# sean-lo/OptimalMatrixCompletion.jl

Measured on AMD Instinct MI355X. Metric: B&B node-relaxations/sec, 100x100 k=1, higher is better.
Workload: dtype f64

## Files before the change

include/omc.h:

```cpp
#ifndef OMC_H
#define OMC_H

#include <stdint.h>

#ifdef __cplusplus
extern "C" {
#endif

#define OMC_VERSION 100

#define OMC_OPTIMAL 0
#define OMC_SLOW_PROGRESS 1
#define OMC_TIME_LIMIT 2
#define OMC_INFEASIBLE 3

#define OMC_CUT_LINEAR 0
#define OMC_CUT_LINEAR2 1
#define OMC_CUT_LINEAR3 2
#define OMC_DIR_LEFT 0
#define OMC_DIR_MIDDLE 1
#define OMC_DIR_RIGHT 2
#define OMC_DIR_INNER_LEFT 3
#define OMC_DIR_INNER_RIGHT 4
#define OMC_SMALLEST_1_EIGVEC 1
// ... 192 lines not shown
int omc_last_kernel_stats(omc_instance* h, int64_t* launches , double* ms ,
                          int64_t* units );
#define OMC_HOST_CHECK_WAIT 0
#define OMC_HOST_CHECK_SCAN 1
#define OMC_HOST_LIST 2
#define OMC_HOST_EVENT_DRAIN 3
#define OMC_HOST_HARVEST_FLAGS 4
#define OMC_HOST_HARVEST_ENQUEUE 5
#define OMC_HOST_HARVEST_WAIT 6
#define OMC_HOST_HARVEST_BOOK 7
#define OMC_HOST_SETUP_ENQUEUE 8
#define OMC_HOST_CHECK_TOTAL 9
#define OMC_HOST_HARVEST_TOTAL 10
#define OMC_HOST_ASYNC_HARVESTS 11
#define OMC_HOST_QUIET_INTERVALS 12
#define OMC_HOST_NPHASE 13
int omc_last_host_phases(omc_instance* h, double* ms , int64_t* count );

#ifdef __cplusplus
}
#endif
#endif
```

optimalmatrixcompletion.jl_amd/api.py:

```python
from __future__ import annotations

import atexit
import weakref
import ctypes as C

import numpy as np

from . import _lib, certificate
from ._lib import RelaxParams, OmcError

CUT_TYPES = {"linear": 0, "linear2": 1, "linear3": 2}
DIR_CODES = {"left": 0, "middle": 1, "right": 2, "inner_left": 3, "inner_right": 4}
BREAKPOINTS = {"smallest_1_eigvec": 1, "smallest_2_eigvec": 2}
STATUS_NAMES = {0: "OPTIMAL", 1: "SLOW_PROGRESS", 2: "TIME_LIMIT", 3: "INFEASIBLE"}
KERNEL_CLASSES = ["colprox", "cone", "global", "check", "setup", "small", "accel", "cone_sub", "check_col", "check_build", "harvest",
                  "shor_bigcone", "shor_minors", "shor_cols"]
HOST_PHASES = ["check_wait", "check_scan", "list", "event_drain", "harvest_flags", "harvest_enqueue", "harvest_wait", "harvest_book",
               "setup_enqueue", "check_total", "harvest_total", "async_harvests", "quiet_intervals"]
RESIDENCY_KERNELS = ["k_cone_sub<0>", "k_cone_sub<1>", "k_cone_sub<2>", "k_global", "k_small", "k_colprox_pair", "k_colprox_wide", "k_colprox",
                     "k_cone_ws", "k_cone"]


def default_params(**kw) -> RelaxParams:
    p = RelaxParams()
    _lib.load().omc_relax_params_default(C.byref(p))
    for k_, v in kw.items():
        if not hasattr(p, k_):
            raise TypeError(f"unknown relaxation parameter {k_!r}")
        setattr(p, k_, v)
    return p


def _pack_cuts(nodes, n, k, cut_type):
# ... 335 lines not shown
            return out
        self.stage(nodes, disjunctive_cuts_type, params, U_lower, U_upper, rho_scales, load_from, save_to)
        self.solve()
        return self.fetch(want_Y, want_X, want_Theta)

    def kernel_stats(self):
        nc = len(KERNEL_CLASSES); la = np.zeros(nc, np.int64); ms = np.zeros(nc); un = np.zeros(nc, np.int64)
        _lib.check(self._lib.omc_last_kernel_stats(self._h, _lib.ptr(la), _lib.ptr(ms), _lib.ptr(un)))
        return {KERNEL_CLASSES[i]: dict(launches=int(la[i]), ms=float(ms[i]), units=int(un[i])) for i in range(nc)}

    def host_phases(self):
        if not hasattr(self._lib, "omc_last_host_phases"):
            raise OmcError(-100, "this build of the library has no omc_last_host_phases")
        ms = np.zeros(len(HOST_PHASES)); cnt = np.zeros(len(HOST_PHASES), np.int64)
        _lib.check(self._lib.omc_last_host_phases(self._h, _lib.ptr(ms), _lib.ptr(cnt)))
        return {HOST_PHASES[i]: dict(ms=float(ms[i]), count=int(cnt[i])) for i in range(len(HOST_PHASES))}

    def subspace_stats(self):
        out = np.zeros(8, np.int64)
        _lib.check(self._lib.omc_last_subspace_stats(self._h, _lib.ptr(out)))
        return dict(calls=int(out[0]), power_steps=int(out[1]), fallbacks=int(out[2]), seeds=int(out[3]), fail_positive=int(out[4]),
                    fail_steps=int(out[5]), fail_cholesky=int(out[6]), ritz_passes=int(out[7]))

    def shor_subspace_stats(self):
        out = np.zeros(8, np.int64)
        _lib.check(self._lib.omc_last_shor_subspace_stats(self._h, _lib.ptr(out)))
        return dict(calls=int(out[0]), power_steps=int(out[1]), fallbacks=int(out[2]), seeds=int(out[3]), fail_positive=int(out[4]),
                    fail_steps=int(out[5]), fail_cholesky=int(out[6]), ritz_passes=int(out[7]))

    def kernel_residency(self):
        out = np.zeros(len(RESIDENCY_KERNELS), np.int32)
# ... 293 lines not shown
```

optimalmatrixcompletion.jl_amd/csrc/omc_host.h:

```cpp
#pragma once
#include <hip/hip_runtime.h>
#include <stdint.h>
#include <atomic>
#include <mutex>
#include <string>
#include <thread>
#include <unordered_map>
#include <vector>

#include "omc.h"
#include "omc_device.h"
#include "omc_shor_relax.h"

extern thread_local std::string g_err;
static inline int fail(int code, const std::string& msg) { g_err = msg; return code; }
#define HIPCHK(x)                                                                                         \
  do {                                                                                                    \
    hipError_t e_ = (x);                                                                                  \
    if (e_ != hipSuccess) {                                                                               \
      g_err = std::string(#x) + ": " + hipGetErrorString(e_);                                             \
      return (int)e_ > 0 ? (int)e_ : 999;                                                                 \
    }                                                                                                     \
  } while (0)

// ... 41 lines not shown
  bool cone_512 = false;
  bool dense_proj = false;
  bool host_phases = false;
  bool global_nolds = false;
  bool no_colprox_pair = false;
  bool no_graph = false;
  bool no_subspace = false;
  bool no_ws_split = false;
  bool segv_trace = false;
  bool setup_gram_inline = false;
  bool shor_explicit = false;
  bool shor_no_subspace = false;
  int check_xs = 16;
  int colprox_block_min = 65;
  int cone_multi_min = 1025;
  int graph_max = 16;
  int harvest_async = 1;
  int harvest_async_min_live = 256;
  int shor_select_kb = 1048576;
  int streams = 4;
  int sub_debug = 0;
  int sub_qmax = 24;
  int timing_stride = 1;
  int ws_quiet = 1;
};
struct Knob { const char* name; bool Tuning::*flag; int Tuning::*num; };
inline const Knob OMC_KNOBS[] = {
  {"OMC_ALTMIN_NOLDS", &Tuning::altmin_nolds, nullptr},      {"OMC_COLPROX_NO_XCD", &Tuning::colprox_no_xcd, nullptr},
  {"OMC_CONE_512", &Tuning::cone_512, nullptr},              {"OMC_DENSE_PROJ", &Tuning::dense_proj, nullptr},
  {"OMC_GLOBAL_NOLDS", &Tuning::global_nolds, nullptr},      {"OMC_HOST_PHASES", &Tuning::host_phases, nullptr},
  {"OMC_NO_COLPROX_PAIR", &Tuning::no_colprox_pair, nullptr},
  {"OMC_NO_GRAPH", &Tuning::no_graph, nullptr},              {"OMC_NO_SUBSPACE", &Tuning::no_subspace, nullptr},
  {"OMC_NO_WS_SPLIT", &Tuning::no_ws_split, nullptr},        {"OMC_SEGV_TRACE", &Tuning::segv_trace, nullptr},
  {"OMC_SETUP_GRAM_INLINE", &Tuning::setup_gram_inline, nullptr},
  {"OMC_SHOR_EXPLICIT", &Tuning::shor_explicit, nullptr},    {"OMC_SHOR_NO_SUBSPACE", &Tuning::shor_no_subspace, nullptr},
  {"OMC_COLPROX_BLOCK_MIN", nullptr, &Tuning::colprox_block_min},
  {"OMC_CHECK_XS", nullptr, &Tuning::check_xs},              {"OMC_CONE_MULTI_MIN", nullptr, &Tuning::cone_multi_min},
  {"OMC_GRAPH_MAX", nullptr, &Tuning::graph_max},            {"OMC_SHOR_SELECT_KB", nullptr, &Tuning::shor_select_kb},
  {"OMC_HARVEST_ASYNC", nullptr, &Tuning::harvest_async},    {"OMC_HARVEST_ASYNC_MIN_LIVE", nullptr, &Tuning::harvest_async_min_live},
  {"OMC_WS_QUIET", nullptr, &Tuning::ws_quiet},
  {"OMC_STREAMS", nullptr, &Tuning::streams},
  {"OMC_SUB_DEBUG", nullptr, &Tuning::sub_debug},            {"OMC_SUB_QMAX", nullptr, &Tuning::sub_qmax},
  {"OMC_TIMING_STRIDE", nullptr, &Tuning::timing_stride},
};

struct omc_instance {
  int n = 0, m = 0, k = 0, device = 0, nnz = 0, cmax = 0;
  double gamma = 0, sumA2 = 0;
  std::vector<int> col_ptr, col_idx; std::vector<double> col_val;
  std::vector<double> A; std::vector<uint8_t> mask;
  std::vector<double> Ncnt;
  std::vector<int> row_ptr, row_idx; std::vector<double> row_val;
// ... 46 lines not shown
      scolpart, sminpart, sminpart2, sfroB, svvB, se1, se2, soX, soW, soTh, sbigscr, sXsB, ssubSB, ssubIB;
  long long big_sub_tot[8] = {0};
  struct ShorListKey { int64_t nq = 0, nsoc = 0; uint64_t hlist = 0; std::vector<int64_t> idx, soc; };
  int64_t reserve_shor_nq = 0; int reserve_shor_lists = 0; bool reserve_shor_set = false;
  std::unordered_map<uint64_t, std::vector<int>> sh_byhash; std::vector<ShorListKey> sh_lists;
  int sh_group_cap = 0; size_t sh_int_used = 0, sh_int_cap = 0, sh_byte_used = 0, sh_byte_cap = 0;
  int pool_cap = 0; DevBuf pY, pD1, pD3, pU, palpha, psval, pXs, ptheta, pscal, bwarmL, bwarmS; std::vector<int> warm_load, warm_save;
  struct PoolSig { int kind = 0; int64_t nq = 0, nsoc = 0; uint64_t hlist = 0, hsoc = 0; };
  bool pool_shor = false; int64_t pool_nqmax = 0; DevBuf pShor, pShorHdr, sloadpart;
  std::vector<PoolSig> pool_sig, node_sig; std::mutex sig_mu;
  std::vector<int> save_host;
  bool shor_warm = false;
  int64_t shor_warm_stats[4] = {0, 0, 0, 0};
  int64_t launches[OMC_KERNEL_NCLASS] = {0}; double ms[OMC_KERNEL_NCLASS] = {0}; int64_t units[OMC_KERNEL_NCLASS] = {0};
  size_t nnz_rows() const { return row_idx.size(); }
  std::vector<hipEvent_t> ev_pool[2]; size_t ev_used[2] = {0, 0}; int ev_cur = 0;
  std::vector<int> ev_class[2];
};

bool next_event_pair(omc_instance* h);
int finish_events(omc_instance* h, int pool);
#define TIMED_ON(strm, cls, counted, units_, call)                                                            \
  do {                                                                                                        \
    const int pc_ = h->ev_cur;                                                                                \
    const bool t0_ = next_event_pair(h) && hipEventRecord(h->ev_pool[pc_][h->ev_used[pc_]], strm) == hipSuccess; \
    call;                                                                                                     \
    if (t0_ && hipEventRecord(h->ev_pool[pc_][h->ev_used[pc_] + 1], strm) == hipSuccess) {                    \
      h->ev_used[pc_] += 2; h->ev_class[pc_].push_back(cls);                                                  \
    }                                                                                                         \
    if (counted) { h->launches[cls] += 1; h->units[cls] += (units_); }                                        \
  } while (0)
#define TIMED(cls, units_, call) TIMED_ON(h->stream, cls, true, units_, call)

static constexpr int MAX_SWEEPS = 30;
```

optimalmatrixcompletion.jl_amd/csrc/omc_relax_solve.cpp:

```cpp
#include <algorithm>
#include <chrono>
#include <stdio.h>

#include "omc_host.h"
#include "omc_slots.h"

static_assert(SLOT_HARVEST_NONE == OMC_HARVEST_NONE && SLOT_HARVEST_SYNC == OMC_HARVEST_SYNC && SLOT_HARVEST_ASYNC == OMC_HARVEST_ASYNC, "omc_slots.h restates the plans of omc.h");

bool next_event_pair(omc_instance* h) {
  std::vector<hipEvent_t>& pool = h->ev_pool[h->ev_cur];
  while (pool.size() < h->ev_used[h->ev_cur] + 2) {
    hipEvent_t e;
    if (hipEventCreate(&e) != hipSuccess) return false;
    pool.push_back(e);
  }
  return true;
}

int finish_events(omc_instance* h, int pool) {
  for (size_t i = 0; i + 1 < h->ev_used[pool]; i += 2) {
    float msv = 0.f;
    if (hipEventElapsedTime(&msv, h->ev_pool[pool][i], h->ev_pool[pool][i + 1]) == hipSuccess) h->ms[h->ev_class[pool][i / 2]] += msv;
  }
  h->ev_used[pool] = 0; h->ev_class[pool].clear();
  return 0;
}

namespace {

using Clock = std::chrono::steady_clock;

int sum_sub_stat(int* sub_stat, int S, long long tot[8], hipStream_t s) {
  std::vector<int> ss(8 * (size_t)S);
  HIPCHK(hipMemcpyAsync(ss.data(), sub_stat, sizeof(int) * ss.size(), hipMemcpyDeviceToHost, s));
  HIPCHK(hipStreamSynchronize(s));
  for (int q = 0; q < 8; ++q) tot[q] = 0;
  for (int b = 0; b < S; ++b) for (int q = 0; q < 8; ++q) tot[q] += ss[8 * b + q];
  HIPCHK(hipMemsetAsync(sub_stat, 0, sizeof(int) * ss.size(), s));
  return 0;
}

struct SolveLoop {
  struct CloseGuard { omc_instance* h; ~CloseGuard() { std::lock_guard<std::mutex> lk(h->append_mu); h->append_closed = true; h->ws.Btot = h->Btot_live.load(); h->Btot = h->ws.Btot; if (h->shor_on) h->sh.Btot = h->ws.Btot; } };
  struct GraphGuard { hipGraphExec_t e[2] = {nullptr, nullptr}; ~GraphGuard() { for (int q = 0; q < 2; ++q) if (e[q]) (void)hipGraphExecDestroy(e[q]); } };

  omc_instance* const h;
  CloseGuard close_guard;
  const OmcWS& w; const ShWS& sw; const omc_relax_params& P;
  const Tuning tun;
  const int S, check_every;
  const bool multi, shor;
  const hipStream_t s;
  hipStream_t sm = nullptr, sb = nullptr, sc = nullptr;
  int Btot;
  int* done = nullptr; int* jobs = nullptr;
  SlotBook book;
  std::vector<int> harvested_ids;
  int harvested = 0, it = 0, nlist = 0, flags_cur = 0, list_cur = 0;
  bool timed_out = false;
  int drain_pool = -1;
  bool wait_main = true;
  bool ev_main_set = false;
  bool mw_any = false; int mw_budget[2] = {MAX_SWEEPS, MAX_SWEEPS};
  bool split_solve = false;
  bool quiet = false, quiet_next = false;
  int graph_max = 0, gexec_n = -1; GraphGuard graphs;
  int nrefilled = 0; bool list_pushed = false;
  const Clock::time_point t0; Clock::time_point t_last, t_check;

  explicit SolveLoop(omc_instance* h_)
      : h(h_), close_guard{h_}, w(h_->ws), sw(h_->sh), P(h_->params), tun(h_->tun), S(h_->ws.B), check_every(std::max(1, h_->params.check_every)),
        multi(h_->tun.streams > 1), shor(h_->shor_on), s(h_->stream), Btot(h_->Btot_live.load()),
        book(h_->ws.B, nullptr, nullptr), t0(Clock::now()), t_last(t0), t_check(t0) {}

  void stamp_begin() { t_last = Clock::now(); }
  void stamp(int q) { const auto t = Clock::now(); h->host_ms[q] += std::chrono::duration<double, std::milli>(t - t_last).count(); h->host_cnt[q] += 1; t_last = t; }
  double elapsed() const { return std::chrono::duration<double>(Clock::now() - t0).count(); }

  int image_free(int q) {
    if (h->ev_up_rec[q]) { HIPCHK(hipEventSynchronize(h->ev_up[q])); h->ev_up_rec[q] = false; }
    return 0;
  }
  int push_flags(bool sync) {
    const int q = flags_cur; flags_cur ^= 1;
    { int rc = image_free(q); if (rc) return rc; }
    int* flags = h->pin_flags[q].as<int>();
    book.write_flags(flags);
    HIPCHK(hipMemcpyAsync(w.node_of, flags, sizeof(int) * 3 * (size_t)S, hipMemcpyHostToDevice, s));
    HIPCHK(hipEventRecord(h->ev_up[q], s)); h->ev_up_rec[q] = true;
    if (sync) HIPCHK(hipStreamSynchronize(s));
    return 0;
  }
  int push_list() {
    const int q = list_cur; list_cur ^= 1;
    { int rc = image_free(2 + q); if (rc) return rc; }
    int* alist = h->pin_list[q].as<int>();
    nlist = book.write_list(alist);
    if (nlist) { HIPCHK(hipMemcpyAsync(h->bslotlist.p, alist, sizeof(int) * nlist, hipMemcpyHostToDevice, s)); HIPCHK(hipEventRecord(h->ev_up[2 + q], s)); h->ev_up_rec[2 + q] = true; }
    return 0;
  }

  int gram_launch(int njobs) {
    if (tun.setup_gram_inline || njobs <= 0) return 0;
    for (int q = 0; q < njobs; ++q)
      if (jobs[2 * q] < 0 || jobs[2 * q] >= S || jobs[2 * q + 1] < 0 || jobs[2 * q + 1] >= Btot) return fail(OMC_ERR_ARGUMENT, "omc_relax_solve: k_setup_gram job outside the slots / nodes");
    HIPCHK(hipMemcpyAsync(h->bgramjobs.p, jobs, sizeof(int) * 2 * (size_t)njobs, hipMemcpyHostToDevice, sb));
    TIMED_ON(sb, OMC_KERNEL_SETUP, false, 0, omc_launch_setup_gram(&w, h->bgramjobs.as<int>(), njobs, Btot, sb));
    HIPCHK(hipEventRecord(h->ev_gram, sb)); h->ev_gram_rec = true;
    return 0;
  }
  int gram_jobs_free() {
    if (h->ev_gram_rec) { HIPCHK(hipEventSynchronize(h->ev_gram)); h->ev_gram_rec = false; }
    return 0;
  }
  int gram_join() {
    if (h->ev_gram_rec && sb != s) HIPCHK(hipStreamWaitEvent(s, h->ev_gram, 0));
    return 0;
  }
  int setup_slots(int units) {
    if (shor) omc_shor_launch_setup(&sw, s);
    TIMED(OMC_KERNEL_SETUP, units, omc_launch_setup(&w, s));
    { int rc = gram_join(); if (rc) return rc; }
    mw_budget[0] = mw_budget[1] = MAX_SWEEPS;
    quiet = quiet_next = false;
    return 0;
  }

  int prepare() {
    for (int c = 0; c < OMC_KERNEL_NCLASS; ++c) { h->launches[c] = 0; h->ms[c] = 0; h->units[c] = 0; }
    for (int q = 0; q < 2; ++q) { h->ev_used[q] = 0; h->ev_class[q].clear(); }
    h->ev_cur = 0;
    for (int q = 0; q < OMC_HOST_NPHASE; ++q) { h->host_ms[q] = 0; h->host_cnt[q] = 0; }
    for (int q = 0; q < 2; ++q) { int rc = h->pin_flags[q].ensure(sizeof(int) * 3 * (size_t)S); if (rc) return rc; rc = h->pin_list[q].ensure(sizeof(int) * (size_t)S); if (rc) return rc; }
    { int rc = h->pin_done.ensure(sizeof(int) * ((size_t)S + 1)); if (rc) return rc; rc = h->pin_jobs.ensure(sizeof(int) * 2 * (size_t)S); if (rc) return rc; rc = h->bgramjobs.ensure(sizeof(int) * 2 * (size_t)S); if (rc) return rc; }
    for (int q = 0; q < 4; ++q) { if (!h->ev_up[q]) HIPCHK(hipEventCreateWithFlags(&h->ev_up[q], hipEventDisableTiming)); h->ev_up_rec[q] = false; }
    if (!h->ev_gram) HIPCHK(hipEventCreateWithFlags(&h->ev_gram, hipEventDisableTiming));
    h->ev_gram_rec = false;
    if (multi && !h->ev_main) {
      for (hipStream_t& q : h->gs) HIPCHK(hipStreamCreateWithFlags(&q, hipStreamNonBlocking));
      for (int q = 0; q < 5; ++q) { HIPCHK(hipEventCreateWithFlags(&h->gev[q], hipEventDisableTiming)); HIPCHK(hipEventCreateWithFlags(&h->gevc[q], hipEventDisableTiming)); }
      HIPCHK(hipEventCreateWithFlags(&h->ev_main, hipEventDisableTiming));
    }
    sm = multi ? h->gs[0] : s; sb = multi ? h->gs[1] : s; sc = multi ? h->gs[2] : s;
    h->ws.setup_gram_inline = tun.setup_gram_inline ? 1 : 0;
    h->ws.check_xs = std::min(std::max(0, tun.check_xs), CB_XS);
    done = h->pin_done.as<int>(); jobs = h->pin_jobs.as<int>();
    book = SlotBook(S, jobs, done);
    int rc = gram_launch(book.start(Btot)); if (rc) return rc;
    rc = push_flags(false); if (rc) return rc;
    if (book.active() < S) { HIPCHK(hipMemcpyAsync(w.done, done, sizeof(int) * S, hipMemcpyHostToDevice, s)); HIPCHK(hipStreamSynchronize(s)); }
    rc = setup_slots(S); if (rc) return rc;
    rc = push_list(); if (rc) return rc;
    h->total_sweeps = 0;
    graph_max = Btot <= tun.graph_max ? tun.graph_max : 0;
    mw_any = w.geo.mw || (shor && h->wbig.geo.mw);
    for (int q = 0; q < 5; ++q) h->mw_tot[q] = 0;
    split_solve = multi && !tun.no_ws_split && w.sub_enable && w.geo.ws_lpp && w.ws_first;
    return 0;
// ... 30 lines not shown
    *ended = false;
    {
      std::lock_guard<std::mutex> lk(h->append_mu);
      Btot = h->Btot_live.load();
      if (timed_out) { int rc = close_unslotted(OMC_ST_TIME); if (rc) return rc; }
      if (book.next_node() >= Btot && (!h->hold.load() || elapsed() > P.time_limit)) { h->append_closed = true; *ended = true; return 0; }
    }
    if (book.next_node() >= Btot) { std::this_thread::sleep_for(std::chrono::microseconds(100)); return 0; }
    return refill_idle();
  }

  int enqueue_body(const OmcWS& wg, bool timed, bool with_aa, bool capturing) {
    const int gact = book.running();
    const bool split = split_solve && (capturing || !quiet);
    hipEvent_t* const ev = capturing ? h->gevc : h->gev;
    if (multi) {
      HIPCHK(hipEventRecord(ev[0], sm));
      HIPCHK(hipStreamWaitEvent(sb, ev[0], 0)); HIPCHK(hipStreamWaitEvent(sc, ev[0], 0));
    }
#define MAYBE_TIMED(strm, cls, units_, call) do { if (timed) TIMED_ON(strm, cls, true, units_, call); else { call; } } while (0)
    if (shor) {
      OmcWS wb = h->wbig; wb.nB = wg.nB; wb.slot_list = wg.slot_list;
      if (w.sub_enable) MAYBE_TIMED(sm, OMC_KERNEL_CONESUB, gact, omc_launch_cone_sub(&wg, sm));
      if (wb.sub_enable) MAYBE_TIMED(sb, OMC_KERNEL_SHOR_BIGCONE, 0, omc_launch_cone_sub(&wb, sb));
      wb.mw_budget = mw_budget[1];
      if (wb.geo.ws_lpp || wb.geo.mw) MAYBE_TIMED(sb, OMC_KERNEL_SHOR_BIGCONE, gact, omc_launch_cone_ws(&wb, sb));
      else MAYBE_TIMED(sb, OMC_KERNEL_SHOR_BIGCONE, gact, omc_launch_cone(&wb, CONE_BIG, sb));
      if (w.geo.ws_lpp || w.geo.mw) MAYBE_TIMED(sm, OMC_KERNEL_CONE, gact, omc_launch_cone_ws(&wg, sm));
      else MAYBE_TIMED(sm, OMC_KERNEL_CONE, gact, omc_launch_cone(&wg, CONE_CLIP01, sm));
      MAYBE_TIMED(sc, OMC_KERNEL_SMALL, gact, omc_launch_small(&wg, SMALL_PROJ, sc));
      MAYBE_TIMED(sc, OMC_KERNEL_SHOR_MINORS, gact, { omc_shor_launch_minor_pre(&sw, sc); omc_shor_launch_vkeys(&sw, sc); });
      if (multi) {
        HIPCHK(hipEventRecord(ev[1], sb)); HIPCHK(hipEventRecord(ev[2], sc));
        HIPCHK(hipStreamWaitEvent(sm, ev[1], 0)); HIPCHK(hipStreamWaitEvent(sm, ev[2], 0));
      }
      MAYBE_TIMED(sm, OMC_KERNEL_GLOBAL, gact, omc_launch_global(&wg, sm));
      MAYBE_TIMED(sm, OMC_KERNEL_SHOR_COLS, gact, omc_shor_launch_cols(&sw, sm));
      MAYBE_TIMED(sm, OMC_KERNEL_SHOR_MINORS, gact, { omc_shor_launch_minor_post(&sw, sm); omc_shor_launch_reduce(&sw, sm); });
      return 0;
    }
    if (split) {
      MAYBE_TIMED(sc, OMC_KERNEL_SMALL, gact, omc_launch_small(&wg, SMALL_PROJ, sc));
      OmcWS wA = wg; wA.ws_phase = 1;
      MAYBE_TIMED(sc, OMC_KERNEL_CONE, gact, omc_launch_cone_ws(&wA, sc));
      HIPCHK(hipEventRecord(ev[4], sc));
    }
    if (w.sub_enable) MAYBE_TIMED(sm, OMC_KERNEL_CONESUB, gact, omc_launch_cone_sub(&wg, sm));
    MAYBE_TIMED(sb, OMC_KERNEL_COLPROX, (int64_t)gact * w.m, omc_launch_colprox(&wg, 0, sb));
    if (split) {
      HIPCHK(hipStreamWaitEvent(sm, ev[4], 0));
      OmcWS wB = wg; wB.ws_phase = 2;
      MAYBE_TIMED(sm, OMC_KERNEL_CONE, 0, omc_launch_cone_ws(&wB, sm));
    }
    else if (w.geo.ws_lpp || w.geo.mw) MAYBE_TIMED(sm, OMC_KERNEL_CONE, gact, omc_launch_cone_ws(&wg, sm));
    else MAYBE_TIMED(sm, OMC_KERNEL_CONE, gact, omc_launch_cone(&wg, CONE_CLIP01, sm));
    if (!split) MAYBE_TIMED(sc, OMC_KERNEL_SMALL, gact, omc_launch_small(&wg, SMALL_PROJ, sc));
    if (multi) {
      HIPCHK(hipEventRecord(ev[1], sb)); HIPCHK(hipEventRecord(ev[2], sc));
      HIPCHK(hipStreamWaitEvent(sm, ev[1], 0)); HIPCHK(hipStreamWaitEvent(sm, ev[2], 0));
    }
    MAYBE_TIMED(sm, OMC_KERNEL_GLOBAL, gact, omc_launch_global(&wg, sm));
    if (with_aa) MAYBE_TIMED(sm, OMC_KERNEL_ACCEL, gact, omc_launch_aa(&wg, sm));
#undef MAYBE_TIMED
    return 0;
  }

  int capture_body(const OmcWS& wg) {
    hipGraphExec_t* const gexec = graphs.e;
    for (int q = 0; q < 2; ++q) { if (gexec[q]) { (void)hipGraphExecDestroy(gexec[q]); gexec[q] = nullptr; } }
    for (int q = 0; q < (w.accel ? 2 : 1); ++q) {
      hipGraph_t gr = nullptr;
      HIPCHK(hipStreamBeginCapture(sm, hipStreamCaptureModeThreadLocal));
      int rc = enqueue_body(wg, false, q == 1, true);
      hipError_t ce = hipStreamEndCapture(sm, &gr);
      if (rc) { if (gr) (void)hipGraphDestroy(gr); return rc; }
      HIPCHK(ce);
      hipError_t ie = hipGraphInstantiate(&gexec[q], gr, nullptr, nullptr, 0);
      (void)hipGraphDestroy(gr);
      HIPCHK(ie);
    }
    gexec_n = nlist;
    return 0;
  }

  int enqueue_iteration(bool* is_check) {
    ++it;
    *is_check = (it % check_every == 0);
    if (multi && wait_main && !ev_main_set) HIPCHK(hipEventRecord(h->ev_main, s));
    ev_main_set = false;
    const bool sampled = tun.timing_stride > 0 && (it % tun.timing_stride) == 0;
    const bool use_graph = multi && nlist <= graph_max && !tun.no_graph && !(sampled && tun.timing_stride > 1) && !mw_any;
    if (book.running() > 0) {
      OmcWS wg = w; wg.slot_list = h->bslotlist.as<int>(); wg.nB = nlist; wg.mw_budget = mw_budget[0];
      if (multi && wait_main) HIPCHK(hipStreamWaitEvent(sm, h->ev_main, 0));
      if (use_graph) {
        if (gexec_n != nlist) { int rc = capture_body(wg); if (rc) return rc; }
        HIPCHK(hipGraphLaunch(graphs.e[(!*is_check && w.accel) ? 1 : 0], sm));
        h->launches[OMC_KERNEL_GLOBAL] += 1; h->units[OMC_KERNEL_GLOBAL] += book.running();
      } else {
        if (quiet && split_solve && (it - 1) % check_every == 0) h->host_cnt[OMC_HOST_QUIET_INTERVALS] += 1;
        int rc = enqueue_body(wg, sampled, !*is_check && w.accel, false); if (rc) return rc;
      }
      if (multi && *is_check) { HIPCHK(hipEventRecord(h->gev[3], sm)); HIPCHK(hipStreamWaitEvent(s, h->gev[3], 0)); }
    }
    wait_main = false;
    if (drain_pool >= 0) {
      stamp_begin(); finish_events(h, drain_pool); drain_pool = -1; stamp(OMC_HOST_EVENT_DRAIN);
    }
    return 0;
  }

  void enqueue_check() {
    const int nactive = book.active();
    wait_main = true;
    timed_out = elapsed() > P.time_limit;
    TIMED(OMC_KERNEL_CHECK_COL, nactive, {
      if (shor) omc_shor_launch_check(&sw, s);
      else { omc_launch_check_zero(&w, s); omc_launch_colprox(&w, 1, s); }
    });
    TIMED(OMC_KERNEL_CHECK_BUILD, nactive, omc_launch_check_build(&w, s));
    TIMED(OMC_KERNEL_CHECK, nactive, {
      if (w.cert_enable) {
        omc_launch_cert_sub(&w, s);
        omc_launch_check_final(&w, timed_out ? OMC_ST_TIME : 0, 0, s);
        OmcWS wc = w; wc.ws_mode = 1; omc_launch_cone_ws(&wc, s);
        omc_launch_check_final(&w, timed_out ? OMC_ST_TIME : 0, 1, s);
      } else {
        if (w.geo.ws_lpp || w.geo.mw) { OmcWS wc = w; wc.ws_mode = 1; omc_launch_cone_ws(&wc, s); }
        else omc_launch_cone(&w, CONE_EVALS, s);
// ... 23 lines not shown
    return 0;
  }

  int read_check() {
    stamp_begin();
    const bool track_quiet = split_solve && tun.ws_quiet && w.ws_need;
    done[S] = 1;
    HIPCHK(hipMemcpyAsync(done, w.done, sizeof(int) * ((size_t)S + (track_quiet ? 1 : 0)), hipMemcpyDeviceToHost, s));
    if (track_quiet) HIPCHK(hipMemsetAsync(w.ws_need, 0, sizeof(int), s));
    HIPCHK(hipStreamSynchronize(s));
    stamp(OMC_HOST_CHECK_WAIT);
    quiet_next = track_quiet && done[S] == 0;
    t_check = t_last;
    nrefilled = 0; list_pushed = false;
    { int rc = mw_collect(); if (rc) return rc; }
    if (drain_pool >= 0) { finish_events(h, drain_pool); drain_pool = -1; }
    drain_pool = h->ev_cur; h->ev_cur ^= 1;
    Btot = h->Btot_live.load();
    if (!P.first_wins) return 0;
    std::vector<int> stv(S);
    HIPCHK(hipMemcpyAsync(stv.data(), w.status, sizeof(int) * S, hipMemcpyDeviceToHost, s));
    HIPCHK(hipStreamSynchronize(s));
    bool won = false;
    for (int b = 0; b < S; ++b) if (book.node(b) >= 0 && done[b] && stv[b] == OMC_ST_OPTIMAL) won = true;
    if (!won) return 0;
    book.finish_all();
    HIPCHK(hipMemcpyAsync(w.done, done, sizeof(int) * S, hipMemcpyHostToDevice, s));
    HIPCHK(hipStreamSynchronize(s));
    return close_unslotted(OMC_ST_SLOW);
  }

  void enqueue_harvest(int nslots) {
    TIMED(OMC_KERNEL_HARVEST, nslots, {
      if (w.save_to) omc_launch_state_save(&w, s);
      if (shor) omc_shor_launch_state_save(&sw, s);
      omc_launch_small(&w, SMALL_RECOVER, s);
      if (w.sep_done) omc_launch_sep_sub(&w, s);
      omc_launch_cone(&w, CONE_SEP, s);
      omc_launch_harvest(&w, s);
      if (w.cert_flag) omc_launch_cert_harvest(&w, s);
      if (shor) omc_shor_launch_harvest(&sw, s);
    });
  }
  void book_harvested() {
    if (w.save_to) {
      std::lock_guard<std::mutex> lk(h->sig_mu);
      for (int id : harvested_ids) {
// ... 12 lines not shown
    nrefilled = book.book_async(Btot, timed_out, harvested_ids);
    book_harvested();
    stamp(OMC_HOST_HARVEST_BOOK);
    rc = gram_launch(nrefilled); if (rc) return rc;
    rc = push_flags(false); if (rc) return rc;
    if (nrefilled) { rc = setup_slots(nrefilled); if (rc) return rc; }
    stamp(OMC_HOST_SETUP_ENQUEUE);
    return 0;
  }

  int harvest_async() {
    const int npend = book.mark_async();
    int rc = push_list(); if (rc) return rc;
    list_pushed = true;
    stamp(OMC_HOST_LIST);
    if (multi) { HIPCHK(hipEventRecord(h->ev_main, s)); ev_main_set = true; }
    rc = push_flags(false); if (rc) return rc;
    stamp(OMC_HOST_HARVEST_FLAGS);
    enqueue_harvest(npend);
    stamp(OMC_HOST_HARVEST_ENQUEUE);
    h->host_cnt[OMC_HOST_ASYNC_HARVESTS] += 1;
    return 0;
  }

  int harvest_sync(int nfin) {
    int rc = gram_jobs_free(); if (rc) return rc;
    rc = gram_launch(book.mark_sync(Btot, timed_out)); if (rc) return rc;
    rc = push_flags(false); if (rc) return rc;
    stamp(OMC_HOST_HARVEST_FLAGS);
    enqueue_harvest(nfin);
    stamp(OMC_HOST_HARVEST_ENQUEUE);
// ... 16 lines not shown
    if (timed_out) { int rc = close_unslotted(OMC_ST_TIME); if (rc) return rc; }
    const int q = harvested_now ? OMC_HOST_HARVEST_TOTAL : OMC_HOST_CHECK_TOTAL;
    h->host_ms[q] += std::chrono::duration<double, std::milli>(Clock::now() - t_check).count(); h->host_cnt[q] += 1;
    return 0;
  }

  int collect_statistics() {
    { int rc = mw_collect(); if (rc) return rc; }
    std::vector<int> sweeps(S);
    HIPCHK(hipMemcpyAsync(sweeps.data(), w.sweeps, sizeof(int) * S, hipMemcpyDeviceToHost, s));
    HIPCHK(hipStreamSynchronize(s));
    for (int v : sweeps) h->total_sweeps += v;
    { int rc = sum_sub_stat(w.sub_stat, S, h->sub_tot, s); if (rc) return rc; }
    if (shor && h->wbig.sub_enable) { int rc = sum_sub_stat(h->wbig.sub_stat, S, h->big_sub_tot, s); if (rc) return rc; }
    HIPCHK(hipGetLastError());
    if (drain_pool >= 0) finish_events(h, drain_pool);
    finish_events(h, h->ev_cur);
    h->last_solve_seconds = elapsed();
    h->last_iters_total = it;
    if (tun.host_phases) {
      static const char* const nm[OMC_HOST_NPHASE] = {"check_wait", "check_scan", "list", "event_drain", "harvest_flags", "harvest_enqueue", "harvest_wait", "harvest_book", "setup_enqueue", "check_total", "harvest_total", "async_harvests", "quiet_intervals"};
      fprintf(stderr, "omc host phases (solve %.1f ms, %d iterations):", 1e3 * h->last_solve_seconds, it);
      for (int q = 0; q < OMC_HOST_NPHASE; ++q) fprintf(stderr, " %s %.3f ms / %lld", nm[q], h->host_ms[q], (long long)h->host_cnt[q]);
      fprintf(stderr, "\n");
    }
    return 0;
  }
};

}

extern "C" {

int omc_cone_multi_budget(int interval_max) { return interval_max > 0 ? std::min(MAX_SWEEPS, interval_max + 2) : MAX_SWEEPS; }

int omc_harvest_plan(int nlive, int nfin, int pending, int check_index, int async_min_live) {
// ... 34 lines not shown
```

Measured before the change: 2265.

## Reuse timing events as cross-stream dependency events via an event tape

Adds an EventTape that tracks the most recent timing event recorded on each stream. Cross-stream joins (fork, side joins, check dependency) wait on that existing event instead of recording a separate sync event, whenever no work has been enqueued on the stream since. This aims to cut the number of hipEventRecord and hipStreamWaitEvent calls per iteration in timed, non-graph bodies. It adds bookkeeping that must call touch() after every enqueue; a missed touch would produce a wrong dependency.

```diff
diff --git a/include/omc.h b/include/omc.h
--- a/include/omc.h
+++ b/include/omc.h
@@ -230,7 +230,9 @@
 #define OMC_HOST_HARVEST_TOTAL 10
 #define OMC_HOST_ASYNC_HARVESTS 11
 #define OMC_HOST_QUIET_INTERVALS 12
-#define OMC_HOST_NPHASE 13
+#define OMC_HOST_BODY_RECORDS 13
+#define OMC_HOST_BODY_WAITS 14
+#define OMC_HOST_NPHASE 15
 int omc_last_host_phases(omc_instance* h, double* ms , int64_t* count );
 
 #ifdef __cplusplus
diff --git a/optimalmatrixcompletion.jl_amd/api.py b/optimalmatrixcompletion.jl_amd/api.py
--- a/optimalmatrixcompletion.jl_amd/api.py
+++ b/optimalmatrixcompletion.jl_amd/api.py
@@ -16,7 +16,8 @@
 KERNEL_CLASSES = ["colprox", "cone", "global", "check", "setup", "small", "accel", "cone_sub", "check_col", "check_build", "harvest",
                   "shor_bigcone", "shor_minors", "shor_cols"]
 HOST_PHASES = ["check_wait", "check_scan", "list", "event_drain", "harvest_flags", "harvest_enqueue", "harvest_wait", "harvest_book",
-               "setup_enqueue", "check_total", "harvest_total", "async_harvests", "quiet_intervals"]
+               "setup_enqueue", "check_total", "harvest_total", "async_harvests", "quiet_intervals", "body_records", "body_waits"]
+HOST_BODY_COUNTS = ("body_records", "body_waits")
 RESIDENCY_KERNELS = ["k_cone_sub<0>", "k_cone_sub<1>", "k_cone_sub<2>", "k_global", "k_small", "k_colprox_pair", "k_colprox_wide", "k_colprox",
                      "k_cone_ws", "k_cone"]
 
@@ -382,7 +383,14 @@
             raise OmcError(-100, "this build of the library has no omc_last_host_phases")
         ms = np.zeros(len(HOST_PHASES)); cnt = np.zeros(len(HOST_PHASES), np.int64)
         _lib.check(self._lib.omc_last_host_phases(self._h, _lib.ptr(ms), _lib.ptr(cnt)))
-        return {HOST_PHASES[i]: dict(ms=float(ms[i]), count=int(cnt[i])) for i in range(len(HOST_PHASES))}
+        return {HOST_PHASES[i]: dict(ms=float(ms[i]), count=int(cnt[i])) for i in range(len(HOST_PHASES)) if HOST_PHASES[i] not in HOST_BODY_COUNTS}
+
+    def event_counts(self):
+        if not hasattr(self._lib, "omc_last_host_phases"):
+            raise OmcError(-100, "this build of the library has no omc_last_host_phases")
+        ms = np.zeros(len(HOST_PHASES)); cnt = np.zeros(len(HOST_PHASES), np.int64)
+        _lib.check(self._lib.omc_last_host_phases(self._h, _lib.ptr(ms), _lib.ptr(cnt)))
+        return {name[len("body_"):]: int(cnt[HOST_PHASES.index(name)]) for name in HOST_BODY_COUNTS}
 
     def subspace_stats(self):
         out = np.zeros(8, np.int64)
diff --git a/optimalmatrixcompletion.jl_amd/csrc/omc_events.h b/optimalmatrixcompletion.jl_amd/csrc/omc_events.h
--- /dev/null
+++ b/optimalmatrixcompletion.jl_amd/csrc/omc_events.h
@@ -0,0 +1,56 @@
+#pragma once
+#include <vector>
+
+template <class Backend>
+class EventTape {
+ public:
+  struct Ev { int pool = -1, index = -1; bool valid() const { return index >= 0; } };
+  struct Launch { int start, stop, cls; };
+
+  EventTape(Backend* be_, int nstreams, bool merge_) : be(be_), merge(merge_), adj(nstreams, -1) {}
+
+  void touch(int stream) { adj[stream] = -1; }
+
+  Ev mark(int stream) {
+    if (merge && adj[stream] >= 0) return Ev{cur, adj[stream]};
+    return fresh(stream);
+  }
+  Ev begin(int stream) { return mark(stream); }
+  Ev end(int stream) { return fresh(stream); }
+
+  bool wait(int stream, Ev e) {
+    const bool ok = be->wait(stream, e.pool, e.index);
+    if (ok) { touch(stream); ++nwaits; }
+    return ok;
+  }
+
+  void launch(Ev start, Ev stop, int cls) { timed[cur].push_back(Launch{start.index, stop.index, cls}); }
+
+  int current() const { return cur; }
+  void swap() { cur ^= 1; for (int& a : adj) a = -1; }
+  const std::vector<Launch>& launches(int pool) const { return timed[pool]; }
+  void drain(int pool) { timed[pool].clear(); used[pool] = 0; if (pool == cur) for (int& a : adj) a = -1; }
+  void reset() { drain(0); drain(1); cur = 0; nrecords = nwaits = 0; }
+
+  long long records() const { return nrecords; }
+  long long waits() const { return nwaits; }
+  void count_record() { ++nrecords; }
+  void count_wait() { ++nwaits; }
+
+ private:
+  Ev fresh(int stream) {
+    const int i = used[cur];
+    if (!be->record(cur, i, stream)) return Ev{};
+    used[cur] = i + 1; ++nrecords;
+    adj[stream] = i;
+    return Ev{cur, i};
+  }
+
+  Backend* be;
+  bool merge;
+  int cur = 0;
+  int used[2] = {0, 0};
+  std::vector<int> adj;
+  std::vector<Launch> timed[2];
+  long long nrecords = 0, nwaits = 0;
+};
diff --git a/optimalmatrixcompletion.jl_amd/csrc/omc_host.h b/optimalmatrixcompletion.jl_amd/csrc/omc_host.h
--- a/optimalmatrixcompletion.jl_amd/csrc/omc_host.h
+++ b/optimalmatrixcompletion.jl_amd/csrc/omc_host.h
@@ -79,6 +79,7 @@
   int check_xs = 16;
   int colprox_block_min = 65;
   int cone_multi_min = 1025;
+  int event_merge = 1;
   int graph_max = 16;
   int harvest_async = 1;
   int harvest_async_min_live = 256;
@@ -101,6 +102,7 @@
   {"OMC_SHOR_EXPLICIT", &Tuning::shor_explicit, nullptr},    {"OMC_SHOR_NO_SUBSPACE", &Tuning::shor_no_subspace, nullptr},
   {"OMC_COLPROX_BLOCK_MIN", nullptr, &Tuning::colprox_block_min},
   {"OMC_CHECK_XS", nullptr, &Tuning::check_xs},              {"OMC_CONE_MULTI_MIN", nullptr, &Tuning::cone_multi_min},
+  {"OMC_EVENT_MERGE", nullptr, &Tuning::event_merge},
   {"OMC_GRAPH_MAX", nullptr, &Tuning::graph_max},            {"OMC_SHOR_SELECT_KB", nullptr, &Tuning::shor_select_kb},
   {"OMC_HARVEST_ASYNC", nullptr, &Tuning::harvest_async},    {"OMC_HARVEST_ASYNC_MIN_LIVE", nullptr, &Tuning::harvest_async_min_live},
   {"OMC_WS_QUIET", nullptr, &Tuning::ws_quiet},
@@ -177,22 +179,7 @@
   int64_t shor_warm_stats[4] = {0, 0, 0, 0};
   int64_t launches[OMC_KERNEL_NCLASS] = {0}; double ms[OMC_KERNEL_NCLASS] = {0}; int64_t units[OMC_KERNEL_NCLASS] = {0};
   size_t nnz_rows() const { return row_idx.size(); }
-  std::vector<hipEvent_t> ev_pool[2]; size_t ev_used[2] = {0, 0}; int ev_cur = 0;
-  std::vector<int> ev_class[2];
+  std::vector<hipEvent_t> ev_pool[2];
 };
 
-bool next_event_pair(omc_instance* h);
-int finish_events(omc_instance* h, int pool);
-#define TIMED_ON(strm, cls, counted, units_, call)                                                            \
-  do {                                                                                                        \
-    const int pc_ = h->ev_cur;                                                                                \
-    const bool t0_ = next_event_pair(h) && hipEventRecord(h->ev_pool[pc_][h->ev_used[pc_]], strm) == hipSuccess; \
-    call;                                                                                                     \
-    if (t0_ && hipEventRecord(h->ev_pool[pc_][h->ev_used[pc_] + 1], strm) == hipSuccess) {                    \
-      h->ev_used[pc_] += 2; h->ev_class[pc_].push_back(cls);                                                  \
-    }                                                                                                         \
-    if (counted) { h->launches[cls] += 1; h->units[cls] += (units_); }                                        \
-  } while (0)
-#define TIMED(cls, units_, call) TIMED_ON(h->stream, cls, true, units_, call)
-
 static constexpr int MAX_SWEEPS = 30;
diff --git a/optimalmatrixcompletion.jl_amd/csrc/omc_relax_solve.cpp b/optimalmatrixcompletion.jl_amd/csrc/omc_relax_solve.cpp
--- a/optimalmatrixcompletion.jl_amd/csrc/omc_relax_solve.cpp
+++ b/optimalmatrixcompletion.jl_amd/csrc/omc_relax_solve.cpp
@@ -2,29 +2,11 @@
 #include <chrono>
 #include <stdio.h>
 
+#include "omc_events.h"
 #include "omc_host.h"
 #include "omc_slots.h"
 
 static_assert(SLOT_HARVEST_NONE == OMC_HARVEST_NONE && SLOT_HARVEST_SYNC == OMC_HARVEST_SYNC && SLOT_HARVEST_ASYNC == OMC_HARVEST_ASYNC, "omc_slots.h restates the plans of omc.h");
-
-bool next_event_pair(omc_instance* h) {
-  std::vector<hipEvent_t>& pool = h->ev_pool[h->ev_cur];
-  while (pool.size() < h->ev_used[h->ev_cur] + 2) {
-    hipEvent_t e;
-    if (hipEventCreate(&e) != hipSuccess) return false;
-    pool.push_back(e);
-  }
-  return true;
-}
-
-int finish_events(omc_instance* h, int pool) {
-  for (size_t i = 0; i + 1 < h->ev_used[pool]; i += 2) {
-    float msv = 0.f;
-    if (hipEventElapsedTime(&msv, h->ev_pool[pool][i], h->ev_pool[pool][i + 1]) == hipSuccess) h->ms[h->ev_class[pool][i / 2]] += msv;
-  }
-  h->ev_used[pool] = 0; h->ev_class[pool].clear();
-  return 0;
-}
 
 namespace {
 
@@ -40,6 +22,32 @@
   return 0;
 }
 
+enum { T_S = 0, T_M = 1, T_B = 2, T_C = 3, T_NSTREAM = 4 };
+struct HipEvents {
+  omc_instance* h; hipStream_t st[T_NSTREAM] = {}; hipError_t last = hipSuccess;
+  bool record(int pool, int i, int stream) {
+    std::vector<hipEvent_t>& p = h->ev_pool[pool];
+    while (p.size() <= (size_t)i) {
+      hipEvent_t e;
+      if ((last = hipEventCreate(&e)) != hipSuccess) return false;
+      p.push_back(e);
+    }
+    return (last = hipEventRecord(p[i], st[stream])) == hipSuccess;
+  }
+  bool wait(int stream, int pool, int i) { return (last = hipStreamWaitEvent(st[stream], h->ev_pool[pool][i], 0)) == hipSuccess; }
+};
+using Tape = EventTape<HipEvents>;
+
+#define TIMED_ON(id, cls, counted, units_, call)                                                          \
+  do {                                                                                                    \
+    const Tape::Ev t0_ = tape.begin(id);                                                                  \
+    call;                                                                                                 \
+    tape.touch(id);                                                                                       \
+    if (t0_.valid()) { const Tape::Ev t1_ = tape.end(id); if (t1_.valid()) tape.launch(t0_, t1_, cls); }  \
+    if (counted) { h->launches[cls] += 1; h->units[cls] += (units_); }                                    \
+  } while (0)
+#define TIMED(cls, units_, call) TIMED_ON(T_S, cls, true, units_, call)
+
 struct SolveLoop {
   struct CloseGuard { omc_instance* h; ~CloseGuard() { std::lock_guard<std::mutex> lk(h->append_mu); h->append_closed = true; h->ws.Btot = h->Btot_live.load(); h->Btot = h->ws.Btot; if (h->shor_on) h->sh.Btot = h->ws.Btot; } };
   struct GraphGuard { hipGraphExec_t e[2] = {nullptr, nullptr}; ~GraphGuard() { for (int q = 0; q < 2; ++q) if (e[q]) (void)hipGraphExecDestroy(e[q]); } };
@@ -52,6 +60,8 @@
   const bool multi, shor;
   const hipStream_t s;
   hipStream_t sm = nullptr, sb = nullptr, sc = nullptr;
+  int im = T_S, ib = T_S, ic = T_S;
+  HipEvents hip_events; Tape tape;
   int Btot;
   int* done = nullptr; int* jobs = nullptr;
   SlotBook book;
@@ -70,12 +80,46 @@
 
   explicit SolveLoop(omc_instance* h_)
       : h(h_), close_guard{h_}, w(h_->ws), sw(h_->sh), P(h_->params), tun(h_->tun), S(h_->ws.B), check_every(std::max(1, h_->params.check_every)),
-        multi(h_->tun.streams > 1), shor(h_->shor_on), s(h_->stream), Btot(h_->Btot_live.load()),
-        book(h_->ws.B, nullptr, nullptr), t0(Clock::now()), t_last(t0), t_check(t0) {}
+        multi(h_->tun.streams > 1), shor(h_->shor_on), s(h_->stream),
+        hip_events{h_}, tape(&hip_events, T_NSTREAM, h_->tun.event_merge != 0), Btot(h_->Btot_live.load()), book(h_->ws.B, nullptr, nullptr), t0(Clock::now()), t_last(t0), t_check(t0) {}
 
   void stamp_begin() { t_last = Clock::now(); }
   void stamp(int q) { const auto t = Clock::now(); h->host_ms[q] += std::chrono::duration<double, std::milli>(t - t_last).count(); h->host_cnt[q] += 1; t_last = t; }
   double elapsed() const { return std::chrono::duration<double>(Clock::now() - t0).count(); }
+
+  void finish_events(int pool) {
+    for (const Tape::Launch& l : tape.launches(pool)) {
+      float msv = 0.f;
+      if (hipEventElapsedTime(&msv, h->ev_pool[pool][l.start], h->ev_pool[pool][l.stop]) == hipSuccess) h->ms[l.cls] += msv;
+    }
+    tape.drain(pool);
+  }
+
+  int depend(int from, int to, int to2, bool on_tape, hipEvent_t fb, bool counted = true) {
+    if (on_tape) {
+      const Tape::Ev e = tape.mark(from);
+      if (e.valid()) {
+        if (!tape.wait(to, e) || (to2 >= 0 && !tape.wait(to2, e))) HIPCHK(hip_events.last);
+        return 0;
+      }
+    }
+    HIPCHK(hipEventRecord(fb, hip_events.st[from])); tape.touch(from); if (counted) tape.count_record();
+    HIPCHK(hipStreamWaitEvent(hip_events.st[to], fb, 0)); tape.touch(to); if (counted) tape.count_wait();
+    if (to2 >= 0) { HIPCHK(hipStreamWaitEvent(hip_events.st[to2], fb, 0)); tape.touch(to2); if (counted) tape.count_wait(); }
+    return 0;
+  }
+  int join_sides(bool on_tape, hipEvent_t fb_b, hipEvent_t fb_c, bool counted) {
+    Tape::Ev eb, ec;
+    if (on_tape) eb = tape.mark(ib);
+    if (!eb.valid()) { HIPCHK(hipEventRecord(fb_b, sb)); tape.touch(ib); if (counted) tape.count_record(); }
+    if (on_tape) ec = tape.mark(ic);
+    if (!ec.valid()) { HIPCHK(hipEventRecord(fb_c, sc)); tape.touch(ic); if (counted) tape.count_record(); }
+    if (eb.valid()) { if (!tape.wait(im, eb)) HIPCHK(hip_events.last); }
+    else { HIPCHK(hipStreamWaitEvent(sm, fb_b, 0)); tape.touch(im); if (counted) tape.count_wait(); }
+    if (ec.valid()) { if (!tape.wait(im, ec)) HIPCHK(hip_events.last); }
+    else { HIPCHK(hipStreamWaitEvent(sm, fb_c, 0)); tape.touch(im); if (counted) tape.count_wait(); }
+    return 0;
+  }
 
   int image_free(int q) {
     if (h->ev_up_rec[q]) { HIPCHK(hipEventSynchronize(h->ev_up[q])); h->ev_up_rec[q] = false; }
@@ -87,6 +131,7 @@
     int* flags = h->pin_flags[q].as<int>();
     book.write_flags(flags);
     HIPCHK(hipMemcpyAsync(w.node_of, flags, sizeof(int) * 3 * (size_t)S, hipMemcpyHostToDevice, s));
+    tape.touch(T_S);
     HIPCHK(hipEventRecord(h->ev_up[q], s)); h->ev_up_rec[q] = true;
     if (sync) HIPCHK(hipStreamSynchronize(s));
     return 0;
@@ -96,6 +141,7 @@
     { int rc = image_free(2 + q); if (rc) return rc; }
     int* alist = h->pin_list[q].as<int>();
     nlist = book.write_list(alist);
+    tape.touch(T_S);
     if (nlist) { HIPCHK(hipMemcpyAsync(h->bslotlist.p, alist, sizeof(int) * nlist, hipMemcpyHostToDevice, s)); HIPCHK(hipEventRecord(h->ev_up[2 + q], s)); h->ev_up_rec[2 + q] = true; }
     return 0;
   }
@@ -105,8 +151,10 @@
     for (int q = 0; q < njobs; ++q)
       if (jobs[2 * q] < 0 || jobs[2 * q] >= S || jobs[2 * q + 1] < 0 || jobs[2 * q + 1] >= Btot) return fail(OMC_ERR_ARGUMENT, "omc_relax_solve: k_setup_gram job outside the slots / nodes");
     HIPCHK(hipMemcpyAsync(h->bgramjobs.p, jobs, sizeof(int) * 2 * (size_t)njobs, hipMemcpyHostToDevice, sb));
-    TIMED_ON(sb, OMC_KERNEL_SETUP, false, 0, omc_launch_setup_gram(&w, h->bgramjobs.as<int>(), njobs, Btot, sb));
+    tape.touch(ib);
+    TIMED_ON(ib, OMC_KERNEL_SETUP, false, 0, omc_launch_setup_gram(&w, h->bgramjobs.as<int>(), njobs, Btot, sb));
     HIPCHK(hipEventRecord(h->ev_gram, sb)); h->ev_gram_rec = true;
+    tape.touch(ib);
     return 0;
   }
   int gram_jobs_free() {
@@ -114,10 +162,11 @@
     return 0;
   }
   int gram_join() {
-    if (h->ev_gram_rec && sb != s) HIPCHK(hipStreamWaitEvent(s, h->ev_gram, 0));
+    if (h->ev_gram_rec && sb != s) { HIPCHK(hipStreamWaitEvent(s, h->ev_gram, 0)); tape.touch(T_S); }
     return 0;
   }
   int setup_slots(int units) {
+    tape.touch(T_S);
     if (shor) omc_shor_launch_setup(&sw, s);
     TIMED(OMC_KERNEL_SETUP, units, omc_launch_setup(&w, s));
     { int rc = gram_join(); if (rc) return rc; }
@@ -128,8 +177,7 @@
 
   int prepare() {
     for (int c = 0; c < OMC_KERNEL_NCLASS; ++c) { h->launches[c] = 0; h->ms[c] = 0; h->units[c] = 0; }
-    for (int q = 0; q < 2; ++q) { h->ev_used[q] = 0; h->ev_class[q].clear(); }
-    h->ev_cur = 0;
+    tape.reset();
     for (int q = 0; q < OMC_HOST_NPHASE; ++q) { h->host_ms[q] = 0; h->host_cnt[q] = 0; }
     for (int q = 0; q < 2; ++q) { int rc = h->pin_flags[q].ensure(sizeof(int) * 3 * (size_t)S); if (rc) return rc; rc = h->pin_list[q].ensure(sizeof(int) * (size_t)S); if (rc) return rc; }
     { int rc = h->pin_done.ensure(sizeof(int) * ((size_t)S + 1)); if (rc) return rc; rc = h->pin_jobs.ensure(sizeof(int) * 2 * (size_t)S); if (rc) return rc; rc = h->bgramjobs.ensure(sizeof(int) * 2 * (size_t)S); if (rc) return rc; }
@@ -142,6 +190,8 @@
       HIPCHK(hipEventCreateWithFlags(&h->ev_main, hipEventDisableTiming));
     }
     sm = multi ? h->gs[0] : s; sb = multi ? h->gs[1] : s; sc = multi ? h->gs[2] : s;
+    if (multi) { im = T_M; ib = T_B; ic = T_C; }
+    hip_events.st[T_S] = s; hip_events.st[T_M] = sm; hip_events.st[T_B] = sb; hip_events.st[T_C] = sc;
     h->ws.setup_gram_inline = tun.setup_gram_inline ? 1 : 0;
     h->ws.check_xs = std::min(std::max(0, tun.check_xs), CB_XS);
     done = h->pin_done.as<int>(); jobs = h->pin_jobs.as<int>();
@@ -202,53 +252,49 @@
     const int gact = book.running();
     const bool split = split_solve && (capturing || !quiet);
     hipEvent_t* const ev = capturing ? h->gevc : h->gev;
-    if (multi) {
-      HIPCHK(hipEventRecord(ev[0], sm));
-      HIPCHK(hipStreamWaitEvent(sb, ev[0], 0)); HIPCHK(hipStreamWaitEvent(sc, ev[0], 0));
-    }
-#define MAYBE_TIMED(strm, cls, units_, call) do { if (timed) TIMED_ON(strm, cls, true, units_, call); else { call; } } while (0)
+    const bool tp = timed && !capturing && tun.event_merge;
+    const bool cnt = !capturing;
+    if (multi) { int rc = depend(im, ib, ic, tp, ev[0], cnt); if (rc) return rc; }
+#define MAYBE_TIMED(id, cls, units_, call) do { if (timed) TIMED_ON(id, cls, true, units_, call); else { call; tape.touch(id); } } while (0)
     if (shor) {
       OmcWS wb = h->wbig; wb.nB = wg.nB; wb.slot_list = wg.slot_list;
-      if (w.sub_enable) MAYBE_TIMED(sm, OMC_KERNEL_CONESUB, gact, omc_launch_cone_sub(&wg, sm));
-      if (wb.sub_enable) MAYBE_TIMED(sb, OMC_KERNEL_SHOR_BIGCONE, 0, omc_launch_cone_sub(&wb, sb));
+      if (w.sub_enable) MAYBE_TIMED(im, OMC_KERNEL_CONESUB, gact, omc_launch_cone_sub(&wg, sm));
+      if (wb.sub_enable) MAYBE_TIMED(ib, OMC_KERNEL_SHOR_BIGCONE, 0, omc_launch_cone_sub(&wb, sb));
       wb.mw_budget = mw_budget[1];
-      if (wb.geo.ws_lpp || wb.geo.mw) MAYBE_TIMED(sb, OMC_KERNEL_SHOR_BIGCONE, gact, omc_launch_cone_ws(&wb, sb));
-      else MAYBE_TIMED(sb, OMC_KERNEL_SHOR_BIGCONE, gact, omc_launch_cone(&wb, CONE_BIG, sb));
-      if (w.geo.ws_lpp || w.geo.mw) MAYBE_TIMED(sm, OMC_KERNEL_CONE, gact, omc_launch_cone_ws(&wg, sm));
-      else MAYBE_TIMED(sm, OMC_KERNEL_CONE, gact, omc_launch_cone(&wg, CONE_CLIP01, sm));
-      MAYBE_TIMED(sc, OMC_KERNEL_SMALL, gact, omc_launch_small(&wg, SMALL_PROJ, sc));
-      MAYBE_TIMED(sc, OMC_KERNEL_SHOR_MINORS, gact, { omc_shor_launch_minor_pre(&sw, sc); omc_shor_launch_vkeys(&sw, sc); });
-      if (multi) {
-        HIPCHK(hipEventRecord(ev[1], sb)); HIPCHK(hipEventRecord(ev[2], sc));
-        HIPCHK(hipStreamWaitEvent(sm, ev[1], 0)); HIPCHK(hipStreamWaitEvent(sm, ev[2], 0));
-      }
-      MAYBE_TIMED(sm, OMC_KERNEL_GLOBAL, gact, omc_launch_global(&wg, sm));
-      MAYBE_TIMED(sm, OMC_KERNEL_SHOR_COLS, gact, omc_shor_launch_cols(&sw, sm));
-      MAYBE_TIMED(sm, OMC_KERNEL_SHOR_MINORS, gact, { omc_shor_launch_minor_post(&sw, sm); omc_shor_launch_reduce(&sw, sm); });
+      if (wb.geo.ws_lpp || wb.geo.mw) MAYBE_TIMED(ib, OMC_KERNEL_SHOR_BIGCONE, gact, omc_launch_cone_ws(&wb, sb));
+      else MAYBE_TIMED(ib, OMC_KERNEL_SHOR_BIGCONE, gact, omc_launch_cone(&wb, CONE_BIG, sb));
+      if (w.geo.ws_lpp || w.geo.mw) MAYBE_TIMED(im, OMC_KERNEL_CONE, gact, omc_launch_cone_ws(&wg, sm));
+      else MAYBE_TIMED(im, OMC_KERNEL_CONE, gact, omc_launch_cone(&wg, CONE_CLIP01, sm));
+      MAYBE_TIMED(ic, OMC_KERNEL_SMALL, gact, omc_launch_small(&wg, SMALL_PROJ, sc));
+      MAYBE_TIMED(ic, OMC_KERNEL_SHOR_MINORS, gact, { omc_shor_launch_minor_pre(&sw, sc); omc_shor_launch_vkeys(&sw, sc); });
+      if (multi) { int rc = join_sides(tp, ev[1], ev[2], cnt); if (rc) return rc; }
+      MAYBE_TIMED(im, OMC_KERNEL_GLOBAL, gact, omc_launch_global(&wg, sm));
+      MAYBE_TIMED(im, OMC_KERNEL_SHOR_COLS, gact, omc_shor_launch_cols(&sw, sm));
+      MAYBE_TIMED(im, OMC_KERNEL_SHOR_MINORS, gact, { omc_shor_launch_minor_post(&sw, sm); omc_shor_launch_reduce(&sw, sm); });
       return 0;
     }
+    Tape::Ev e4;
     if (split) {
-      MAYBE_TIMED(sc, OMC_KERNEL_SMALL, gact, omc_launch_small(&wg, SMALL_PROJ, sc));
+      MAYBE_TIMED(ic, OMC_KERNEL_SMALL, gact, omc_launch_small(&wg, SMALL_PROJ, sc));
       OmcWS wA = wg; wA.ws_phase = 1;
-      MAYBE_TIMED(sc, OMC_KERNEL_CONE, gact, omc_launch_cone_ws(&wA, sc));
-      HIPCHK(hipEventRecord(ev[4], sc));
-    }
-    if (w.sub_enable) MAYBE_TIMED(sm, OMC_KERNEL_CONESUB, gact, omc_launch_cone_sub(&wg, sm));
-    MAYBE_TIMED(sb, OMC_KERNEL_COLPROX, (int64_t)gact * w.m, omc_launch_colprox(&wg, 0, sb));
+      MAYBE_TIMED(ic, OMC_KERNEL_CONE, gact, omc_launch_cone_ws(&wA, sc));
+      if (tp) e4 = tape.mark(ic);
+      if (!e4.valid()) { HIPCHK(hipEventRecord(ev[4], sc)); tape.touch(ic); if (cnt) tape.count_record(); }
+    }
+    if (w.sub_enable) MAYBE_TIMED(im, OMC_KERNEL_CONESUB, gact, omc_launch_cone_sub(&wg, sm));
+    MAYBE_TIMED(ib, OMC_KERNEL_COLPROX, (int64_t)gact * w.m, omc_launch_colprox(&wg, 0, sb));
     if (split) {
-      HIPCHK(hipStreamWaitEvent(sm, ev[4], 0));
+      if (e4.valid()) { if (!tape.wait(im, e4)) HIPCHK(hip_events.last); }
+      else { HIPCHK(hipStreamWaitEvent(sm, ev[4], 0)); tape.touch(im); if (cnt) tape.count_wait(); }
       OmcWS wB = wg; wB.ws_phase = 2;
-      MAYBE_TIMED(sm, OMC_KERNEL_CONE, 0, omc_launch_cone_ws(&wB, sm));
-    }
-    else if (w.geo.ws_lpp || w.geo.mw) MAYBE_TIMED(sm, OMC_KERNEL_CONE, gact, omc_launch_cone_ws(&wg, sm));
-    else MAYBE_TIMED(sm, OMC_KERNEL_CONE, gact, omc_launch_cone(&wg, CONE_CLIP01, sm));
-    if (!split) MAYBE_TIMED(sc, OMC_KERNEL_SMALL, gact, omc_launch_small(&wg, SMALL_PROJ, sc));
-    if (multi) {
-      HIPCHK(hipEventRecord(ev[1], sb)); HIPCHK(hipEventRecord(ev[2], sc));
-      HIPCHK(hipStreamWaitEvent(sm, ev[1], 0)); HIPCHK(hipStreamWaitEvent(sm, ev[2], 0));
-    }
-    MAYBE_TIMED(sm, OMC_KERNEL_GLOBAL, gact, omc_launch_global(&wg, sm));
-    if (with_aa) MAYBE_TIMED(sm, OMC_KERNEL_ACCEL, gact, omc_launch_aa(&wg, sm));
+      MAYBE_TIMED(im, OMC_KERNEL_CONE, 0, omc_launch_cone_ws(&wB, sm));
+    }
+    else if (w.geo.ws_lpp || w.geo.mw) MAYBE_TIMED(im, OMC_KERNEL_CONE, gact, omc_launch_cone_ws(&wg, sm));
+    else MAYBE_TIMED(im, OMC_KERNEL_CONE, gact, omc_launch_cone(&wg, CONE_CLIP01, sm));
+    if (!split) MAYBE_TIMED(ic, OMC_KERNEL_SMALL, gact, omc_launch_small(&wg, SMALL_PROJ, sc));
+    if (multi) { int rc = join_sides(tp, ev[1], ev[2], cnt); if (rc) return rc; }
+    MAYBE_TIMED(im, OMC_KERNEL_GLOBAL, gact, omc_launch_global(&wg, sm));
+    if (with_aa) MAYBE_TIMED(im, OMC_KERNEL_ACCEL, gact, omc_launch_aa(&wg, sm));
 #undef MAYBE_TIMED
     return 0;
   }
@@ -274,26 +320,30 @@
   int enqueue_iteration(bool* is_check) {
     ++it;
     *is_check = (it % check_every == 0);
-    if (multi && wait_main && !ev_main_set) HIPCHK(hipEventRecord(h->ev_main, s));
+    if (multi && wait_main && !ev_main_set) { HIPCHK(hipEventRecord(h->ev_main, s)); tape.touch(T_S); }
     ev_main_set = false;
+    const long long nrec0 = tape.records(), nwait0 = tape.waits();
     const bool sampled = tun.timing_stride > 0 && (it % tun.timing_stride) == 0;
     const bool use_graph = multi && nlist <= graph_max && !tun.no_graph && !(sampled && tun.timing_stride > 1) && !mw_any;
     if (book.running() > 0) {
       OmcWS wg = w; wg.slot_list = h->bslotlist.as<int>(); wg.nB = nlist; wg.mw_budget = mw_budget[0];
-      if (multi && wait_main) HIPCHK(hipStreamWaitEvent(sm, h->ev_main, 0));
+      if (multi && wait_main) { HIPCHK(hipStreamWaitEvent(sm, h->ev_main, 0)); tape.count_wait(); }
+      if (wait_main) tape.touch(im);
       if (use_graph) {
         if (gexec_n != nlist) { int rc = capture_body(wg); if (rc) return rc; }
         HIPCHK(hipGraphLaunch(graphs.e[(!*is_check && w.accel) ? 1 : 0], sm));
+        tape.touch(im);
         h->launches[OMC_KERNEL_GLOBAL] += 1; h->units[OMC_KERNEL_GLOBAL] += book.running();
       } else {
         if (quiet && split_solve && (it - 1) % check_every == 0) h->host_cnt[OMC_HOST_QUIET_INTERVALS] += 1;
         int rc = enqueue_body(wg, sampled, !*is_check && w.accel, false); if (rc) return rc;
       }
-      if (multi && *is_check) { HIPCHK(hipEventRecord(h->gev[3], sm)); HIPCHK(hipStreamWaitEvent(s, h->gev[3], 0)); }
-    }
+      if (multi && *is_check) { int rc = depend(im, T_S, -1, sampled && !use_graph && tun.event_merge, h->gev[3]); if (rc) return rc; }
+    }
+    h->host_cnt[OMC_HOST_BODY_RECORDS] += tape.records() - nrec0; h->host_cnt[OMC_HOST_BODY_WAITS] += tape.waits() - nwait0;
     wait_main = false;
     if (drain_pool >= 0) {
-      stamp_begin(); finish_events(h, drain_pool); drain_pool = -1; stamp(OMC_HOST_EVENT_DRAIN);
+      stamp_begin(); finish_events(drain_pool); drain_pool = -1; stamp(OMC_HOST_EVENT_DRAIN);
     }
     return 0;
   }
@@ -301,6 +351,7 @@
   void enqueue_check() {
     const int nactive = book.active();
     wait_main = true;
+    tape.touch(T_S);
     timed_out = elapsed() > P.time_limit;
     TIMED(OMC_KERNEL_CHECK_COL, nactive, {
       if (shor) omc_shor_launch_check(&sw, s);
@@ -354,8 +405,8 @@
     t_check = t_last;
     nrefilled = 0; list_pushed = false;
     { int rc = mw_collect(); if (rc) return rc; }
-    if (drain_pool >= 0) { finish_events(h, drain_pool); drain_pool = -1; }
-    drain_pool = h->ev_cur; h->ev_cur ^= 1;
+    if (drain_pool >= 0) { finish_events(drain_pool); drain_pool = -1; }
+    drain_pool = tape.current(); tape.swap();
     Btot = h->Btot_live.load();
     if (!P.first_wins) return 0;
     std::vector<int> stv(S);
@@ -371,6 +422,7 @@
   }
 
   void enqueue_harvest(int nslots) {
+    tape.touch(T_S);
     TIMED(OMC_KERNEL_HARVEST, nslots, {
       if (w.save_to) omc_launch_state_save(&w, s);
       if (shor) omc_shor_launch_state_save(&sw, s);
@@ -413,7 +465,7 @@
     int rc = push_list(); if (rc) return rc;
     list_pushed = true;
     stamp(OMC_HOST_LIST);
-    if (multi) { HIPCHK(hipEventRecord(h->ev_main, s)); ev_main_set = true; }
+    if (multi) { HIPCHK(hipEventRecord(h->ev_main, s)); ev_main_set = true; tape.touch(T_S); }
     rc = push_flags(false); if (rc) return rc;
     stamp(OMC_HOST_HARVEST_FLAGS);
     enqueue_harvest(npend);
@@ -460,12 +512,12 @@
     { int rc = sum_sub_stat(w.sub_stat, S, h->sub_tot, s); if (rc) return rc; }
     if (shor && h->wbig.sub_enable) { int rc = sum_sub_stat(h->wbig.sub_stat, S, h->big_sub_tot, s); if (rc) return rc; }
     HIPCHK(hipGetLastError());
-    if (drain_pool >= 0) finish_events(h, drain_pool);
-    finish_events(h, h->ev_cur);
+    if (drain_pool >= 0) finish_events(drain_pool);
+    finish_events(tape.current());
     h->last_solve_seconds = elapsed();
     h->last_iters_total = it;
     if (tun.host_phases) {
-      static const char* const nm[OMC_HOST_NPHASE] = {"check_wait", "check_scan", "list", "event_drain", "harvest_flags", "harvest_enqueue", "harvest_wait", "harvest_book", "setup_enqueue", "check_total", "harvest_total", "async_harvests", "quiet_intervals"};
+      static const char* const nm[OMC_HOST_NPHASE] = {"check_wait", "check_scan", "list", "event_drain", "harvest_flags", "harvest_enqueue", "harvest_wait", "harvest_book", "setup_enqueue", "check_total", "harvest_total", "async_harvests", "quiet_intervals", "body_records", "body_waits"};
       fprintf(stderr, "omc host phases (solve %.1f ms, %d iterations):", 1e3 * h->last_solve_seconds, it);
       for (int q = 0; q < OMC_HOST_NPHASE; ++q) fprintf(stderr, " %s %.3f ms / %lld", nm[q], h->host_ms[q], (long long)h->host_cnt[q]);
       fprintf(stderr, "\n");
```

New measurement: 2340 (median of 6 runs). +3.3%, better.
